# SelvinSelbaraju/hm-retrieval-two-tower

Measured on AMD Instinct MI355X. Metric: positive pairs/sec (train) + index QPS @ Recall@100, 1/2/4/8 MI355X, higher is better.
Workload: dtype bf16; 1 GPU; C3: main.py schema @ emb 128, towers [256]->128, logQ in-batch softmax, Adagrad, batch 16384; global_batch=16384, parallelism=dp1

## Files before the change

### hm-retrieval-two-tower_amd/csrc/tt_sparse.hip

```cpp
#include <algorithm>
#include <cstdlib>
#include <cstring>
#include <rocprim/device/device_radix_sort.hpp>

#include "tt_common.h"

namespace tt {
namespace {

template <char OP>
__device__ __forceinline__ float ieee_op(float a, float b) {
  if constexpr (OP == '+') return a + b;
  if constexpr (OP == '-') return a - b;
  if constexpr (OP == '*') return a * b;
  return a / b;
}

constexpr int kBlock = 32;
constexpr int kTablesPerLaunch = 16;
constexpr int kThreads = 256;
constexpr int kPFJoin = 32;
constexpr int64_t kMaxLookups = int64_t(1) << 24;
constexpr int kSrcShift = 28;

constexpr uint32_t kHdrMagic = 0x54545350u;
constexpr int kHdrBytes = 256;
enum : uint32_t { kErrStaleKeys = 1u, kErrOutOfCall = 2u };
struct SparseHeader {
  uint32_t magic;
  uint32_t error;
  uint32_t fp0, fp1;
};

struct TableDesc {
  const int32_t* ids[TT_MAX_SOURCES];
  int32_t goff[TT_MAX_SOURCES];
  const float* grad;
  int32_t gld;
  float* table;
  float* slot0;
  float* slot1;
  int64_t num_rows;
  int32_t dim;
  int32_t num_sources;
  int32_t n;
  int32_t base;
  int32_t n_pad;
  int32_t lanes;
  int32_t wave_begin;
  int32_t chunk_begin;
  int64_t piece_off;
};

struct Job {
  TableDesc t[kTablesPerLaunch];
  int32_t num;
  int32_t id_bits;
  int64_t batch;
  uint32_t* keys_in;
  uint32_t* vals_in;
  const uint32_t* keys;
  const uint32_t* vals;
  float* pieces;
  uint32_t* chunk_hist;
  int32_t num_chunks;
  float* dense_out;
  int32_t dense_dim;
  SparseHeader* hdr;
  uint32_t fp0, fp1;
};

__device__ __forceinline__ bool keys_are_mine(const Job& j) {
  const uint32_t f0 = __builtin_amdgcn_readfirstlane(__hip_atomic_load(&j.hdr->fp0, __ATOMIC_RELAXED,
                                                                        __HIP_MEMORY_SCOPE_AGENT));
  const uint32_t f1 = __builtin_amdgcn_readfirstlane(__hip_atomic_load(&j.hdr->fp1, __ATOMIC_RELAXED,
                                                                        __HIP_MEMORY_SCOPE_AGENT));
  if (f0 == j.fp0 && f1 == j.fp1) return true;
  if (lane_id() == 0) atomicOr(&j.hdr->error, kErrStaleKeys);
  return false;
}

enum ApplyOp { kWriteSum = 0, kAdagrad = 1, kAdamScatter = 2, kScatterSum = 3 };

struct ApplyParams {
  float lr;
  float eps;
  float one_minus_beta1;
  float one_minus_beta2;
};

__device__ __forceinline__ int table_of_wave(const Job& j, int gw) {
  int t = 0;
#pragma unroll 1
  for (int i = 1; i < j.num; ++i)
    if (gw >= j.t[i].wave_begin) t = i;
  return t;
}

__global__ void __launch_bounds__(kThreads) build_keys_kernel(const Job j, int total) {
  const int i = blockIdx.x * kThreads + threadIdx.x;
  if (i >= total) return;
  int t = 0;
#pragma unroll 1
  for (int k = 1; k < j.num; ++k)
    if (i >= j.t[k].base) t = k;
  const TableDesc& T = j.t[t];
  const int loc = i - T.base;
  const uint32_t invalid = (1u << j.id_bits) - 1u;
  uint32_t id = invalid, val = 0xFFFFFFFFu;
  if (loc < T.n) {
    const int s = static_cast<int>(loc / j.batch);
    const int64_t b = loc - s * j.batch;
    const int32_t r = T.ids[s][b];
    const bool ok = r >= 0 && r < T.num_rows;
    id = ok ? static_cast<uint32_t>(r) : invalid;
    val = ok ? (static_cast<uint32_t>(s) << kSrcShift) | static_cast<uint32_t>(b) : 0xFFFFFFFFu;
  }
  j.keys_in[i] = (static_cast<uint32_t>(t) << j.id_bits) | id;
  j.vals_in[i] = val;
  if (i == 0) {
    if (j.hdr->magic != kHdrMagic) {
      j.hdr->error = 0u;
      j.hdr->magic = kHdrMagic;
    }
    j.hdr->fp0 = j.fp0;
    j.hdr->fp1 = j.fp1;
  }
}

constexpr int kLdsSortMax = 16384;
constexpr int kLsThreads = 1024;
constexpr int kLsWaves = kLsThreads / kWave;
constexpr int kLsTiles = kLdsSortMax / kLsWaves / kWave;
constexpr int kHistStride = kLsWaves + 1;
constexpr int kLsLdsBytes = kLdsSortMax * 4 + 2 * kLdsSortMax * 2 + 256 * kHistStride * 4;

struct Region {
  const int32_t *ids0, *ids1, *ids2, *ids3;
  int64_t batch;
  uint32_t* keys;
  uint32_t* vals;
  int n;
  uint32_t nr;
  uint32_t khi;
  uint32_t invalid;
};

__device__ __forceinline__ int source_of(const Region& R, int64_t i) {
  return (i >= R.batch) + (i >= 2 * R.batch) + (i >= 3 * R.batch);
}

__device__ __forceinline__ uint32_t region_key(const Region& R, int i) {
// ... 91 lines not shown
  for (int u = 0; u < 4; ++u) {
    hist[hist_word(4 * tid + u)] = ex;
    ex += h[u];
  }
  __syncthreads();
}

__global__ void __launch_bounds__(kLsThreads) region_sort_kernel(const Job j) {
  extern __shared__ __attribute__((aligned(16))) char lsm[];
  uint32_t* lkey = reinterpret_cast<uint32_t*>(lsm);
  uint16_t* const pbuf0 = reinterpret_cast<uint16_t*>(lsm + kLdsSortMax * 4);
  uint16_t* const pbuf1 = pbuf0 + kLdsSortMax;
  uint32_t* hist = reinterpret_cast<uint32_t*>(lsm + kLdsSortMax * 8);
  __shared__ uint32_t wsum[kLsWaves];
  const int tid = threadIdx.x, lane = lane_id(), w = tid / kWave;
  Region R;
  int n;
  {
    const TableDesc& T = j.t[blockIdx.x];
    R.ids0 = T.ids[0];
    R.ids1 = T.ids[1];
    R.ids2 = T.ids[2];
    R.ids3 = T.ids[3];
    R.batch = j.batch;
    R.keys = const_cast<uint32_t*>(j.keys) + T.base;
    R.vals = const_cast<uint32_t*>(j.vals) + T.base;
    R.n = T.n;
    R.nr = static_cast<uint32_t>(T.num_rows);
    R.khi = static_cast<uint32_t>(blockIdx.x) << j.id_bits;
    R.invalid = (1u << j.id_bits) - 1u;
    n = T.n_pad;
  }
  const uint32_t nr = R.nr;
  if (blockIdx.x == 0 && tid == 0) {
    if (j.hdr->magic != kHdrMagic) {
      j.hdr->error = 0u;
      j.hdr->magic = kHdrMagic;
    }
    j.hdr->fp0 = j.fp0;
    j.hdr->fp1 = j.fp1;
  }
  const int bits = 32 - __builtin_clz(nr);
  const int per = ((n + kLsWaves - 1) / kLsWaves + kWave - 1) / kWave * kWave;
  const int wbeg = w * per, wend = min(n, wbeg + per);
  const uint64_t lt = (uint64_t(1) << lane) - 1u;
  for (int e = tid; e < 256 * kHistStride; e += kLsThreads) hist[e] = 0u;
  if (bits <= 8) {
    uint8_t* k8 = reinterpret_cast<uint8_t*>(lsm);
    const bool staged = n <= kLdsSortMax * 8;
    if (staged) stage_keys(R, n, k8);
    __syncthreads();
    for (int t0 = wbeg; t0 < wend; t0 += kWave) {
      const int i = t0 + lane;
      const bool act = i < wend;
      const uint32_t d = act ? (staged ? k8[i] : region_key(R, i)) : 0u;
      count_peers(hist, d, digit_peers(d, act, bits), w);
    }
    scan_digit_counts(hist, wsum);
    for (int t0 = wbeg; t0 < wend; t0 += kWave) {
      const int i = t0 + lane;
      const bool act = i < wend;
      const uint32_t d = act ? (staged ? k8[i] : region_key(R, i)) : 0u;
      const uint64_t m = digit_peers(d, act, bits);
      if (act) {
        uint32_t* slot = &hist[d * kHistStride + w];
        const uint32_t off = *slot;
// ... 101 lines not shown
    run += h[u];
  }
  uint32_t inc = run;
#pragma unroll
  for (int o = 1; o < kWave; o <<= 1) {
    const uint32_t y = __shfl_up(inc, o, kWave);
    if (lane >= o) inc += y;
  }
  if (lane == kWave - 1) wsum[w] = inc;
  __syncthreads();
  uint32_t ex = inc - run;
  for (int v = 0; v < w; ++v) ex += wsum[v];
#pragma unroll
  for (int u = 0; u < 4; ++u) {
    const int L = 4 * tid + u;
    hist[(L / kCsWaves) * kCsHistStride + L % kCsWaves] = ex;
    ex += h[u];
  }
  __syncthreads();
}

__global__ void __launch_bounds__(kCsThreads) chunk_sort_kernel(const Job j) {
  __shared__ uint32_t lkey[kChunk];
  __shared__ uint16_t pbuf[2][kChunk];
  __shared__ uint32_t hist[256 * kCsHistStride];
  __shared__ uint32_t wsum[kCsWaves];
  const int tid = threadIdx.x, lane = lane_id(), w = tid / kWave;
  const int t = table_of_chunk(j, blockIdx.x);
  const Region R = region_of(j, t);
  const int c0 = (static_cast<int>(blockIdx.x) - j.t[t].chunk_begin) * kChunk;
  const int n = min(kChunk, j.t[t].n_pad - c0);
  uint32_t* ck = j.keys_in + j.t[t].base + c0;
  uint32_t* cp = j.vals_in + j.t[t].base + c0;
  if (blockIdx.x == 0 && tid == 0) {
    if (j.hdr->magic != kHdrMagic) {
      j.hdr->error = 0u;
      j.hdr->magic = kHdrMagic;
    }
    j.hdr->fp0 = j.fp0;
    j.hdr->fp1 = j.fp1;
  }
  {
    uint32_t k[kCsTiles];
#pragma unroll
    for (int u = 0; u < kCsTiles; ++u) k[u] = region_key(R, c0 + u * kCsThreads + tid);
#pragma unroll
    for (int u = 0; u < kCsTiles; ++u) {
      const int i = u * kCsThreads + tid;
      if (i < n) {
        lkey[i] = k[u];
        pbuf[0][i] = static_cast<uint16_t>(i);
      }
    }
  }
  for (int e = tid; e < 256 * kCsHistStride; e += kCsThreads) hist[e] = 0u;
  const int bits = 32 - __builtin_clz(R.nr);
  const int per = ((n + kCsWaves - 1) / kCsWaves + kWave - 1) / kWave * kWave;
  const int wbeg = w * per, wend = min(n, wbeg + per);
  const uint64_t lt = (uint64_t(1) << lane) - 1u;
  const int passes = (bits + 7) / 8;
  const int width = (bits + passes - 1) / passes;
  const uint32_t dmask = (1u << width) - 1u;
  int cur = 0;
  for (int p = 0; p < passes; ++p) {
    const int sh = p * width;
    if (p > 0)
// ... 142 lines not shown
}

struct RowState {
  float x0, x1;
};

template <int OP>
__device__ __forceinline__ RowState load_row(const TableDesc& T, int64_t o) {
  RowState r{0.0f, 0.0f};
  if (OP == kAdagrad) {
    r.x0 = T.slot0[o];
    r.x1 = T.table[o];
  } else if (OP == kAdamScatter) {
    r.x0 = T.slot0[o];
    r.x1 = T.slot1[o];
  }
  return r;
}

template <int OP>
__device__ __forceinline__ void store_row(const TableDesc& T, const ApplyParams& ap, int64_t o, RowState r, float g) {
  if (OP == kAdagrad) {
    const float a = ieee_op<'+'>(r.x0, ieee_op<'*'>(g, g));
    T.slot0[o] = a;
    T.table[o] = ieee_op<'-'>(r.x1, ieee_op<'/'>(ieee_op<'*'>(ap.lr, g), ieee_op<'+'>(sqrtf(a), ap.eps)));
  } else if (OP == kAdamScatter) {
    T.slot0[o] = ieee_op<'+'>(r.x0, ieee_op<'*'>(g, ap.one_minus_beta1));
    T.slot1[o] = ieee_op<'+'>(r.x1, ieee_op<'*'>(ieee_op<'*'>(g, g), ap.one_minus_beta2));
  } else if (OP == kScatterSum) {
    T.table[o] = g;
  }
}

template <int OP>
__device__ __forceinline__ void apply_row(const Job& j, const TableDesc& T, const ApplyParams& ap, uint32_t key,
                                          int seg_start_sorted, int col, float g) {
  const uint32_t id = key & ((1u << j.id_bits) - 1u);
  if (OP == kWriteSum) {
    j.dense_out[static_cast<int64_t>(seg_start_sorted) * j.dense_dim + col] = g;
    return;
  }
  if (id >= static_cast<uint32_t>(T.num_rows)) return;
  const int64_t o = static_cast<int64_t>(id) * T.dim + col;
  store_row<OP>(T, ap, o, load_row<OP>(T, o), g);
}

template <int OP>
__global__ void __launch_bounds__(kThreads) block_sum_kernel(const Job j, const ApplyParams ap) {
  const int gw = __builtin_amdgcn_readfirstlane(static_cast<int>(blockIdx.x * (kThreads / kWave) + threadIdx.x / kWave));
  const int t = table_of_wave(j, gw);
  const TableDesc& T = j.t[t];
  const int P = T.lanes;
  const int lane = lane_id();
  const int blk = (gw - T.wave_begin) * (kWave / P) + lane / P;
  const int nblk = T.n_pad / kBlock;
  if (blk >= nblk) return;
  const int b0 = T.base + blk * kBlock;
  const int tend = T.base + T.n_pad;
  const uint32_t id_mask = (1u << j.id_bits) - 1u;
  uint32_t key[kBlock], off[kBlock];
#pragma unroll
  for (int r = 0; r < kBlock; ++r) {
    key[r] = j.keys[b0 + r];
    off[r] = j.vals[b0 + r];
  }
  const uint32_t kprev = blk > 0 ? j.keys[b0 - 1] : ~0u;
  const uint32_t knext = b0 + kBlock < tend ? j.keys[b0 + kBlock] : ~0u;
  if (!keys_are_mine(j)) return;
  const uint32_t gld = static_cast<uint32_t>(T.gld);
  const uint32_t go0 = T.goff[0], go1 = T.goff[1], go2 = T.goff[2], go3 = T.goff[3];
  const float* __restrict__ grad = T.grad;
  uint32_t ends = 0, apply = 0;
  bool out_of_call = false;
#pragma unroll
  for (int r = 0; r < kBlock; ++r) {
    const uint32_t s = off[r] >> kSrcShift;
    const uint32_t b = off[r] & ((1u << kSrcShift) - 1u);
    const uint32_t o = b * gld + (s == 0 ? go0 : s == 1 ? go1 : s == 2 ? go2 : go3);
    const bool in = s < static_cast<uint32_t>(T.num_sources) && b < static_cast<uint32_t>(j.batch);
    out_of_call = out_of_call || (off[r] != 0xFFFFFFFFu && !in);
    off[r] = (off[r] != 0xFFFFFFFFu && in) ? o : 0xFFFFFFFFu;
    if (r == kBlock - 1 || key[r + 1] != key[r]) ends |= 1u << r;
  }
  if (out_of_call) {
    atomicOr(&j.hdr->error, kErrOutOfCall);
    return;
  }
  const bool head_cont = key[0] == kprev;
  const bool tail_cont = key[kBlock - 1] == knext;
  {
    int seg_begin = 0;
#pragma unroll
    for (int r = 0; r < kBlock; ++r) {
      if (ends >> r & 1u) {
        const bool piece = (seg_begin == 0 && head_cont) || (r == kBlock - 1 && tail_cont);
        const bool valid = OP == kWriteSum || (key[r] & id_mask) < static_cast<uint32_t>(T.num_rows);
        if (!piece && valid) apply |= 1u << r;
        seg_begin = r + 1;
      }
    }
  }
  float* pc = j.pieces + T.piece_off + static_cast<int64_t>(blk) * 2 * T.dim;
  for (int col = lane % P; col < T.dim; col += P) {
    float v[kBlock];
#pragma unroll
    for (int r = 0; r < kBlock; ++r) v[r] = off[r] != 0xFFFFFFFFu ? grad[off[r] + col] : 0.0f;
    float acc = 0.0f;
    int seg_begin = 0;
#pragma unroll
    for (int r = 0; r < kBlock; ++r) {
      acc = ieee_op<'+'>(acc, v[r]);
      v[r] = acc;
      if (ends >> r & 1u) {
        if (seg_begin == 0 && head_cont) pc[col] = acc;
        else if (r == kBlock - 1 && tail_cont) pc[T.dim + col] = acc;
        acc = 0.0f;
        seg_begin = r + 1;
      }
    }
    if (OP == kWriteSum) {
      int sb = 0;
#pragma unroll
      for (int r = 0; r < kBlock; ++r) {
        if (apply >> r & 1u) j.dense_out[static_cast<int64_t>(b0 + sb) * j.dense_dim + col] = ieee_op<'+'>(0.0f, v[r]);
        if (ends >> r & 1u) sb = r + 1;
      }
    } else {
      RowState st[kBlock];
#pragma unroll
      for (int r = 0; r < kBlock; ++r)
        if (apply >> r & 1u) st[r] = load_row<OP>(T, static_cast<int64_t>(key[r] & id_mask) * T.dim + col);
      __builtin_amdgcn_s_waitcnt(0x0F70);
#pragma unroll
      for (int r = 0; r < kBlock; ++r)
        if (apply >> r & 1u)
          store_row<OP>(T, ap, static_cast<int64_t>(key[r] & id_mask) * T.dim + col, st[r], ieee_op<'+'>(0.0f, v[r]));
    }
  }
}

template <int OP>
__global__ void __launch_bounds__(kThreads) join_kernel(const Job j, const ApplyParams ap) {
  const int gw = __builtin_amdgcn_readfirstlane(static_cast<int>(blockIdx.x * (kThreads / kWave) + threadIdx.x / kWave));
  const int t = table_of_wave(j, gw);
  const TableDesc& T = j.t[t];
  const int P = T.lanes;
  const int lane = lane_id();
  const int blk = (gw - T.wave_begin) * (kWave / P) + lane / P;
  const int nblk = T.n_pad / kBlock;
  if (blk >= nblk) return;
  const int b0 = T.base + blk * kBlock;
  const int tend = T.base + T.n_pad;
  const uint32_t klast = j.keys[b0 + kBlock - 1];
  const uint32_t knext = b0 + kBlock < tend ? j.keys[b0 + kBlock] : ~0u;
  const bool mine = keys_are_mine(j);
  if (!mine || knext != klast) return;
  uint32_t key[kBlock];
#pragma unroll
  for (int r = 0; r < kBlock; ++r) key[r] = j.keys[b0 + r];
  const uint32_t kprev = blk > 0 ? j.keys[b0 - 1] : ~0u;
  if ((klast & ((1u << j.id_bits) - 1u)) >= static_cast<uint32_t>(T.num_rows)) return;
  int seg_start = kBlock - 1;
#pragma unroll
  for (int r = kBlock - 2; r >= 0; --r)
    if (key[r] == klast && seg_start == r + 1) seg_start = r;
  if (seg_start == 0 && kprev == klast) return;
  int lo = b0 + kBlock, hi = tend;
  {
    const int li = lane % P, g0 = lane - li;
    const uint64_t gmask = (P == kWave) ? ~0ull : (((1ull << P) - 1ull) << g0);
    while (hi - lo > 1) {
      const int step = (hi - lo + P) / (P + 1);
      const int p = lo + (li + 1) * step;
      const bool eq = p < hi && j.keys[p] == klast;
      const int c = __popcll(__ballot(eq) & gmask);
      const int nlo = lo + c * step;
      if (c < P && lo + (c + 1) * step < hi) hi = lo + (c + 1) * step;
      lo = nlo;
    }
  }
  const int last = (lo - T.base) / kBlock;
  const float* pcs = j.pieces + T.piece_off;
  for (int col = lane % P; col < T.dim; col += P) {
    float g = ieee_op<'+'>(0.0f, pcs[static_cast<int64_t>(blk) * 2 * T.dim + T.dim + col]);
    for (int bb = blk + 1; bb <= last; bb += kPFJoin) {
      float v[kPFJoin];
#pragma unroll
      for (int q = 0; q < kPFJoin; ++q)
        v[q] = (bb + q <= last) ? pcs[static_cast<int64_t>(bb + q) * 2 * T.dim + col] : 0.0f;
#pragma unroll
      for (int q = 0; q < kPFJoin; ++q)
        if (bb + q <= last) g = ieee_op<'+'>(g, v[q]);
    }
    apply_row<OP>(j, T, ap, klast, b0 + seg_start, col, g);
  }
}

__global__ void __launch_bounds__(1024) compact_kernel(const Job j, int32_t* out_uniq, float* out_sum,
                                                       int32_t* out_count) {
  const TableDesc& T = j.t[0];
  __shared__ int scratch[17];
  const int n = T.n_pad;
  const uint32_t mask = (1u << j.id_bits) - 1u;
  const int per = (n + 1023) / 1024;
  const int r0 = threadIdx.x * per, r1 = min(r0 + per, n);
  int heads = 0;
  for (int i = r0; i < r1; ++i) {
    const uint32_t k = j.keys[i];
    if ((k & mask) < static_cast<uint32_t>(T.num_rows) && (i == 0 || j.keys[i - 1] != k)) ++heads;
  }
  const int lane = lane_id(), w = threadIdx.x / kWave;
  int x = heads;
#pragma unroll
  for (int off = 1; off < kWave; off <<= 1) {
    const int y = __shfl_up(x, off, kWave);
    if (lane >= off) x += y;
  }
  if (lane == kWave - 1) scratch[w] = x;
  __syncthreads();
  if (threadIdx.x == 0) {
    int run = 0;
    for (int i = 0; i < 16; ++i) {
      const int tt = scratch[i];
      scratch[i] = run;
      run += tt;
    }
    scratch[16] = run;
// ... 42 lines not shown
  for (int i = 0; i < cnt; ++i) max_rows = std::max<int64_t>(max_rows, tables[i].num_rows);
  j.id_bits = bits_for(max_rows);
  const int table_bits = bits_for(std::max(cnt - 1, 1));
  p->end_bit = j.id_bits + table_bits;
  if (p->end_bit > 32) return fail(TT_ERR_UNSUPPORTED, "sparse: %d tables x %lld rows exceed 32-bit keys", cnt,
                                   static_cast<long long>(max_rows));
  int base = 0, waves = 0, chunks = 0;
  int64_t poff = 0;
  for (int i = 0; i < cnt; ++i) {
    const tt_sparse_table& s = tables[i];
    TableDesc& T = j.t[i];
    for (int q = 0; q < TT_MAX_SOURCES; ++q) {
      T.ids[q] = (q < s.num_sources) ? s.ids[q] : nullptr;
      T.goff[q] = (q < s.num_sources) ? s.grad_col_offset[q] : 0;
    }
    T.grad = s.grad ? s.grad : grad;
    T.gld = static_cast<int32_t>(s.grad ? s.grad_ld : grad_stride);
    if (batch > 0 && !T.grad && !size_query) return fail(TT_ERR_BAD_ARG, "sparse: table %d has no gradient (NULL grad)", i);
    int32_t max_off = 0;
    for (int q = 0; q < s.num_sources; ++q) max_off = std::max(max_off, s.grad_col_offset[q]);
    const int64_t gld = s.grad ? s.grad_ld : grad_stride;
    if (gld < 0 || max_off < 0 || (batch > 0 && (batch - 1) * gld + max_off + s.dim >= (int64_t(1) << 31)))
      return fail(TT_ERR_UNSUPPORTED, "sparse: table %d gradient rows exceed 2^31 floats", i);
    T.table = s.table;
    T.slot0 = s.slot0;
    T.slot1 = s.slot1;
    T.num_rows = s.num_rows;
    T.dim = s.dim;
    T.num_sources = s.num_sources;
    T.n = static_cast<int32_t>(s.num_sources * batch);
    T.base = base;
    T.n_pad = static_cast<int32_t>(round_up(std::max<int64_t>(T.n, 1), kBlock));
    T.lanes = lanes_per_slot(s.dim);
    T.wave_begin = waves;
    T.chunk_begin = chunks;
    T.piece_off = poff;
    base += T.n_pad;
    chunks += static_cast<int>(ceil_div(T.n_pad, kChunk));
    const int nblk = T.n_pad / kBlock;
    waves += static_cast<int>(ceil_div(nblk, kWave / T.lanes));
    poff += static_cast<int64_t>(nblk) * 2 * s.dim;
  }
  p->total = base;
  p->waves = waves;
  j.num_chunks = chunks;
  p->piece_floats = poff;
  uint32_t h0 = 2166136261u, h1 = 0x9747b28cu;
  auto mix = [&](uint64_t v) {
    for (int b = 0; b < 8; ++b) {
      const uint32_t byte = static_cast<uint32_t>(v >> (8 * b)) & 0xFFu;
      h0 = (h0 ^ byte) * 16777619u;
      h1 = (h1 ^ (byte + 0x5bu)) * 0x01000193u + 0x3c6ef372u;
    }
  };
  mix(static_cast<uint64_t>(batch));
  mix(static_cast<uint64_t>(cnt));
  for (int i = 0; i < cnt; ++i) {
    const tt_sparse_table& s = tables[i];
    mix(reinterpret_cast<uintptr_t>(s.table));
    mix(static_cast<uint64_t>(s.num_rows));
    mix((static_cast<uint64_t>(s.dim) << 32) | static_cast<uint32_t>(s.num_sources));
    for (int q = 0; q < s.num_sources; ++q) mix(reinterpret_cast<uintptr_t>(s.ids[q]));
  }
  j.fp0 = h0;
  j.fp1 = h1;
  size_t sb = 0;
  uint32_t* np = nullptr;
  hipError_t e = rocprim::radix_sort_pairs<SortConfig>(nullptr, sb, np, np, np, np, static_cast<unsigned>(base), 0, p->end_bit,
                                           nullptr, false);
  p->sort_bytes = (e == hipSuccess) ? sb : static_cast<size_t>(base) * 8 + (size_t(4) << 20);
  return TT_OK;
}

struct PlanWs {
  SparseHeader* hdr;
  uint32_t *keys_in, *vals_in, *keys, *vals;
  float* pieces;
  uint32_t* chunk_hist;
  float* dense_out;
  void* sort_tmp;
};
PlanWs carve_plan(Carver& cv, const Plan& p, int dense_dim) {
  PlanWs w;
  w.hdr = reinterpret_cast<SparseHeader*>(cv.take<char>(kHdrBytes));
  w.keys_in = cv.take<uint32_t>(p.total);
  w.vals_in = cv.take<uint32_t>(p.total);
  w.keys = cv.take<uint32_t>(p.total);
  w.vals = cv.take<uint32_t>(p.total);
  w.pieces = cv.take<float>(std::max<int64_t>(p.piece_floats, 1));
  w.chunk_hist = cv.take<uint32_t>(static_cast<int64_t>(p.job.num_chunks) * 256);
  w.dense_out = dense_dim > 0 ? cv.take<float>(static_cast<int64_t>(p.total) * dense_dim) : nullptr;
  w.sort_tmp = cv.take<char>(static_cast<int64_t>(p.sort_bytes) + 256);
  return w;
}

int validate_tables(const tt_sparse_table* tables, int32_t num_tables, int64_t batch, bool adam,
                    bool need_slot0 = true) {
  TT_REQUIRE(tables != nullptr && num_tables >= 1, "sparse: no tables");
  TT_REQUIRE(batch >= 0, "sparse: negative batch");
  int64_t total = 0;
  for (int i = 0; i < num_tables; ++i) {
    const tt_sparse_table& t = tables[i];
    TT_REQUIRE(t.table && (t.slot0 || !need_slot0), "sparse: table %d has NULL parameter/slot pointer", i);
    TT_REQUIRE(!adam || t.slot1, "sparse: table %d needs slot1 for Adam", i);
    TT_REQUIRE(t.num_rows >= 1 && t.num_rows < (int64_t(1) << 30), "sparse: table %d num_rows out of range", i);
    TT_REQUIRE(t.dim >= 1 && t.dim <= 4096, "sparse: table %d dim=%d out of range", i, t.dim);
    TT_REQUIRE(t.num_sources >= 1 && t.num_sources <= TT_MAX_SOURCES, "sparse: table %d num_sources=%d", i,
               t.num_sources);
    for (int s = 0; s < t.num_sources; ++s) TT_REQUIRE(t.ids[s] || batch == 0, "sparse: table %d source %d ids NULL", i, s);
    total += t.num_sources * batch;
  }
  TT_REQUIRE(total < kMaxLookups, "sparse: %lld lookups in one call (max %lld)", static_cast<long long>(total),
             static_cast<long long>(kMaxLookups));
  return TT_OK;
}

size_t tables_ws_bytes(const tt_sparse_table* tables, int32_t num_tables, int64_t batch, int dense_dim) {
  size_t total = 0;
  for (int first = 0; first < num_tables; first += kTablesPerLaunch) {
    const int cnt = std::min(num_tables - first, kTablesPerLaunch);
    Plan p;
    if (make_plan(tables + first, cnt, batch, nullptr, 0, &p, true)) return 0;
// ... 10 lines not shown
    const char* e = std::getenv("TT_SPARSE_SORT");
    if (e && std::strcmp(e, "device") == 0) return int(kSortDevice);
    if (e && std::strcmp(e, "region") == 0) return int(kSortRegion);
    return int(kSortChunk);
  }();
  return v;
}

enum SparseStage { kStageAll = 0, kStageSort = 1, kStageApply = 2 };

template <int OP>
int run_sparse(const tt_sparse_table* tables, int32_t num_tables, int64_t batch, const float* grad,
               int64_t grad_stride, const ApplyParams& ap, void* workspace, size_t ws_bytes, hipStream_t st,
               int32_t* out_uniq = nullptr, float* out_sum = nullptr, int32_t* out_count = nullptr,
               int stage = kStageAll) {
  TT_REQUIRE(batch < (int64_t(1) << kSrcShift), "sparse: batch %lld too large", static_cast<long long>(batch));
  TT_REQUIRE(stage == kStageAll || num_tables <= kTablesPerLaunch,
             "sparse: a split sort/apply call takes at most %d tables", kTablesPerLaunch);
  for (int first = 0; first < num_tables; first += kTablesPerLaunch) {
    const int cnt = std::min(num_tables - first, kTablesPerLaunch);
    Plan p;
    int rc = make_plan(tables + first, cnt, batch, grad, grad_stride, &p, stage == kStageSort);
    if (rc) return rc;
    Carver cv(workspace, ws_bytes);
    const int dense_dim = (OP == kWriteSum) ? tables[first].dim : 0;
    PlanWs w = carve_plan(cv, p, dense_dim);
    if (cv.used() > ws_bytes) return fail(TT_ERR_WORKSPACE, "sparse: workspace %zu < required %zu", ws_bytes, cv.used());
    Job& j = p.job;
    j.keys_in = w.keys_in;
    j.vals_in = w.vals_in;
    j.keys = w.keys;
    j.vals = w.vals;
    j.pieces = w.pieces;
    j.chunk_hist = w.chunk_hist;
    j.dense_out = w.dense_out;
    j.dense_dim = dense_dim;
    j.hdr = w.hdr;
    if (stage != kStageApply) {
      const int mode = sort_mode();
      bool lds = mode != kSortDevice, chunked = mode == kSortChunk;
      int merge_chunks = 0;
      for (int i = 0; i < cnt; ++i) {
        const bool small = bits_for(j.t[i].num_rows) <= 8;
        lds = lds && (j.t[i].n_pad <= kLdsSortMax || small);
        chunked = chunked && (small ? j.t[i].n_pad <= kChunkMaxSmall : j.t[i].n_pad <= kChunkMaxLarge);
        if (!small) merge_chunks = std::max(merge_chunks, static_cast<int>(ceil_div(j.t[i].n_pad, kChunk)));
      }
      if (chunked) {
        hipLaunchKernelGGL(chunk_sort_kernel, dim3(j.num_chunks), dim3(kCsThreads), 0, st, j);
        TT_CHECK_LAUNCH();
        static const hipError_t attr = hipFuncSetAttribute(reinterpret_cast<const void*>(chunk_merge_kernel),
                                                           hipFuncAttributeMaxDynamicSharedMemorySize, kMergeLdsMax);
        TT_CHECK_HIP(attr);
        hipLaunchKernelGGL(chunk_merge_kernel, dim3(j.num_chunks), dim3(kCsThreads), merge_chunks * kChunk * 4, st,
                           j);
        TT_CHECK_LAUNCH();
      } else if (lds) {
        static const hipError_t attr = hipFuncSetAttribute(reinterpret_cast<const void*>(region_sort_kernel),
                                                           hipFuncAttributeMaxDynamicSharedMemorySize, kLsLdsBytes);
        TT_CHECK_HIP(attr);
        hipLaunchKernelGGL(region_sort_kernel, dim3(cnt), dim3(kLsThreads), kLsLdsBytes, st, j);
        TT_CHECK_LAUNCH();
      } else {
        hipLaunchKernelGGL(build_keys_kernel, dim3(ceil_div(p.total, kThreads)), dim3(kThreads), 0, st, j, p.total);
        TT_CHECK_LAUNCH();
        size_t sb = p.sort_bytes;
        TT_CHECK_HIP(rocprim::radix_sort_pairs<SortConfig>(w.sort_tmp, sb, w.keys_in, w.keys, w.vals_in, w.vals,
                                               static_cast<unsigned>(p.total), 0, p.end_bit, st, false));
      }
    }
    if (stage == kStageSort) continue;
    const int blocks = static_cast<int>(ceil_div(p.waves, kThreads / kWave));
    hipLaunchKernelGGL(block_sum_kernel<OP>, dim3(blocks), dim3(kThreads), 0, st, j, ap);
    TT_CHECK_LAUNCH();
    hipLaunchKernelGGL(join_kernel<OP>, dim3(blocks), dim3(kThreads), 0, st, j, ap);
    TT_CHECK_LAUNCH();
    if (OP == kWriteSum) {
      hipLaunchKernelGGL(compact_kernel, dim3(1), dim3(1024), 0, st, j, out_uniq, out_sum, out_count);
      TT_CHECK_LAUNCH();
    }
  }
  return TT_OK;
}

__global__ void scale2_kernel(float* a, float sa, float* b, float sb, int64_t n) {
  for (int64_t i = blockIdx.x * (int64_t)blockDim.x + threadIdx.x; i < n; i += (int64_t)gridDim.x * blockDim.x) {
    a[i] = ieee_op<'*'>(a[i], sa);
    b[i] = ieee_op<'*'>(b[i], sb);
  }
}

__global__ void adam_var_kernel(float* var, const float* m, const float* v, float lr, float eps, int64_t n) {
  for (int64_t i = blockIdx.x * (int64_t)blockDim.x + threadIdx.x; i < n; i += (int64_t)gridDim.x * blockDim.x)
    var[i] = ieee_op<'-'>(var[i], ieee_op<'/'>(ieee_op<'*'>(lr, m[i]), ieee_op<'+'>(sqrtf(v[i]), eps)));
}

__global__ void dense_adagrad_kernel(float* p, float* acc, const float* g, int64_t n, float lr, float eps) {
  for (int64_t i = blockIdx.x * (int64_t)blockDim.x + threadIdx.x; i < n; i += (int64_t)gridDim.x * blockDim.x) {
    const float gi = g[i];
    const float a = ieee_op<'+'>(acc[i], ieee_op<'*'>(gi, gi));
    acc[i] = a;
    p[i] = ieee_op<'-'>(p[i], ieee_op<'/'>(ieee_op<'*'>(gi, lr), ieee_op<'+'>(sqrtf(a), eps)));
  }
}

constexpr int kDenseMaxJobs = 8;
struct DenseJobs {
  float* p[kDenseMaxJobs];
  float* acc[kDenseMaxJobs];
// ... 123 lines not shown
    for (int q = 0; q < w; ++q) ex += wsum[q];
    if (tid < r.world) pre[tid * T + t] = ex;
  }
  __syncthreads();
  const int64_t i = static_cast<int64_t>(blockIdx.x) * kRoutedThreads + tid;
  const uint32_t invalid = (1u << j.id_bits) - 1u;
  if (i < r.total) {
    const int lk = r.order[i];
    const int l = static_cast<int>(lk / j.batch);
    const int b = static_cast<int>(lk - static_cast<int64_t>(l) * j.batch);
    const int s = r.slot[lk];
    const int o = s >= 0 ? static_cast<int>(s / r.cap) : -1 - s;
    const int g = o * T + r.lk_tag[l];
    const int dst = r.lk_base[l] + pre[g] + static_cast<int>(i - r.grp_first[g]);
    uint32_t id = s >= 0 ? static_cast<uint32_t>(s) : invalid;
    if (r.slot_row && s >= 0) {
      const int32_t row = r.slot_row[s];
      id = row >= 0 ? static_cast<uint32_t>(row) : invalid;
    }
    const_cast<uint32_t*>(j.keys)[dst] = r.lk_khi[l] | id;
    const_cast<uint32_t*>(j.vals)[dst] = id == invalid ? 0xFFFFFFFFu : (r.lk_shi[l] | static_cast<uint32_t>(b));
  } else {
    const int k = static_cast<int>(i - r.total);
    int t = 0;
#pragma unroll 1
    for (int q = 1; q < r.num_tables; ++q)
      if (k >= r.pad_begin[q]) t = q;
    if (k < r.pad_begin[r.num_tables]) {
      const int dst = r.pad_dst[t] + (k - r.pad_begin[t]);
      const_cast<uint32_t*>(j.keys)[dst] = r.pad_key[t];
      const_cast<uint32_t*>(j.vals)[dst] = 0xFFFFFFFFu;
    }
  }
  if (i == 0) {
    if (j.hdr->magic != kHdrMagic) {
      j.hdr->error = 0u;
      j.hdr->magic = kHdrMagic;
    }
    j.hdr->fp0 = j.fp0;
    j.hdr->fp1 = j.fp1;
  }
}

dim3 stride_grid(int64_t n) {
  int64_t b = ceil_div(n, 256);
  if (b > 8192) b = 8192;
  if (b < 1) b = 1;
  return dim3(static_cast<unsigned>(b));
}

}
}

using namespace tt;

extern "C" size_t tt_sparse_workspace_size(const tt_sparse_table* tables, int32_t num_tables, int64_t batch) {
  if (!tables || num_tables < 1 || batch < 0) return 0;
  return tables_ws_bytes(tables, num_tables, batch, 0);
}

namespace tt {
namespace {
int sparse_adagrad_stage(const tt_sparse_table* tables, int32_t num_tables, int64_t batch, const float* grad,
                         int64_t grad_stride, float lr, float epsilon, void* workspace, size_t workspace_bytes,
                         tt_stream_t stream, int stage, const char* name) {
  clear_error();
// ... 241 lines not shown
  TT_REQUIRE(L >= 1 && L <= kRoutedMaxLookups, "tt_sparse_routed: 1..%d lookups, got %d", kRoutedMaxLookups, L);
  TT_REQUIRE(W >= 1 && W <= kRoutedThreads && T >= 1 && static_cast<int64_t>(W) * T <= kRoutedMaxGroups,
             "tt_sparse_routed: world %d x tags %d out of range", W, T);
  TT_REQUIRE(rs->cap >= 1, "tt_sparse_routed: cap must be >= 1");
  int tag_of_table[kTablesPerLaunch], seen[kTablesPerLaunch][TT_MAX_SOURCES] = {};
  for (int t = 0; t < num_tables; ++t) tag_of_table[t] = -1;
  for (int l = 0; l < L; ++l) {
    const int t = rs->lookup_table[l], s = rs->lookup_source[l], g = rs->lookup_tag[l];
    TT_REQUIRE(t >= 0 && t < num_tables && s >= 0 && s < tables[t].num_sources && g >= 0 && g < T,
               "tt_sparse_routed: lookup %d maps to table %d source %d tag %d: out of range", l, t, s, g);
    TT_REQUIRE(tag_of_table[t] < 0 || tag_of_table[t] == g, "tt_sparse_routed: table %d takes two tags", t);
    TT_REQUIRE(!seen[t][s], "tt_sparse_routed: table %d source %d listed twice", t, s);
    tag_of_table[t] = g;
    seen[t][s] = 1;
  }
  for (int t = 0; t < num_tables; ++t)
    for (int s = 0; s < tables[t].num_sources; ++s)
      TT_REQUIRE(seen[t][s], "tt_sparse_routed: table %d source %d has no routed lookup", t, s);
  for (int t = 0; t < num_tables; ++t)
    for (int u = t + 1; u < num_tables; ++u)
      TT_REQUIRE(tag_of_table[t] != tag_of_table[u], "tt_sparse_routed: tables %d and %d take one tag", t, u);
  const size_t need = tables_ws_bytes(tables, num_tables, batch, 0);
  if (!workspace || workspace_bytes < need)
    return fail(TT_ERR_WORKSPACE, "tt_sparse_routed: workspace %zu < required %zu", workspace_bytes, need);
  TT_REQUIRE(batch < (int64_t(1) << kSrcShift), "tt_sparse_routed: batch too large");
  Plan p;
  rc = make_plan(tables, num_tables, batch, grad, grad_stride, &p);
  if (rc) return rc;
  Carver cv(workspace, workspace_bytes);
  PlanWs w = carve_plan(cv, p, 0);
  Job& j = p.job;
  j.keys = w.keys;
  j.vals = w.vals;
  j.hdr = w.hdr;
  RoutedArgs a{};
  a.order = rs->order;
  a.grp_first = rs->grp_first;
  a.grp_last = rs->grp_last;
  a.slot = rs->slot;
  a.slot_row = rs->slot_row;
  a.cap = rs->cap;
  a.total = static_cast<int64_t>(L) * batch;
  a.world = W;
  a.num_tags = T;
  a.num_lookups = L;
  a.num_tables = num_tables;
  for (int l = 0; l < L; ++l) {
    const int t = rs->lookup_table[l];
    a.lk_tag[l] = rs->lookup_tag[l];
    a.lk_khi[l] = static_cast<uint32_t>(t) << j.id_bits;
    a.lk_shi[l] = static_cast<uint32_t>(rs->lookup_source[l]) << kSrcShift;
    a.lk_base[l] = j.t[t].base;
  }
  int pads = 0;
  for (int t = 0; t < num_tables; ++t) {
    a.pad_begin[t] = pads;
    a.pad_dst[t] = j.t[t].base + j.t[t].n;
    a.pad_key[t] = (static_cast<uint32_t>(t) << j.id_bits) | ((1u << j.id_bits) - 1u);
    pads += j.t[t].n_pad - j.t[t].n;
  }
  a.pad_begin[num_tables] = pads;
  TT_REQUIRE(a.total + pads == p.total, "tt_sparse_routed: %lld routed lookups + %d padding != %d sorted entries",
             static_cast<long long>(a.total), pads, p.total);
  hipStream_t st = to_stream(stream);
  hipLaunchKernelGGL(routed_keys_kernel, dim3(static_cast<unsigned>(ceil_div(p.total, kRoutedThreads))),
                     dim3(kRoutedThreads), 0, st, j, a);
// ... 28 lines not shown
```

Measured before the change: 32.03 million positive pairs/s.

## Fuse cross-block segment join into block_sum via arrival counters

Removes the separate join_kernel launch. Segments that span several 32-row blocks are now finished by whichever block arrives last, tracked with per-block atomic arrival counters that are reset in the key-building and sort kernels. The segment-extent search runs forward and backward at once. Wave assignment now puts small tables (<=255 rows) first, presumably so their long, contended segments start early. This saves a kernel launch and a full pass over keys, but adds atomics, relaxed-memory publish/read of partial sums, and a new workspace array, with some risk around memory ordering.

```diff
diff --git a/hm-retrieval-two-tower_amd/csrc/tt_sparse.hip b/hm-retrieval-two-tower_amd/csrc/tt_sparse.hip
--- a/hm-retrieval-two-tower_amd/csrc/tt_sparse.hip
+++ b/hm-retrieval-two-tower_amd/csrc/tt_sparse.hip
@@ -20,6 +20,8 @@
 constexpr int kTablesPerLaunch = 16;
 constexpr int kThreads = 256;
 constexpr int kPFJoin = 32;
+constexpr int kPFShort = 4;
+constexpr int kSmallRows = 255;
 constexpr int64_t kMaxLookups = int64_t(1) << 24;
 constexpr int kSrcShift = 28;
 
@@ -62,6 +64,7 @@
   const uint32_t* keys;
   const uint32_t* vals;
   float* pieces;
+  uint32_t* arrived;
   uint32_t* chunk_hist;
   int32_t num_chunks;
   float* dense_out;
@@ -90,10 +93,15 @@
 };
 
 __device__ __forceinline__ int table_of_wave(const Job& j, int gw) {
-  int t = 0;
+  int t = 0, best = -1;
 #pragma unroll 1
-  for (int i = 1; i < j.num; ++i)
-    if (gw >= j.t[i].wave_begin) t = i;
+  for (int i = 0; i < j.num; ++i) {
+    const int wb = j.t[i].wave_begin;
+    if (gw >= wb && wb > best) {
+      t = i;
+      best = wb;
+    }
+  }
   return t;
 }
 
@@ -118,6 +126,7 @@
   }
   j.keys_in[i] = (static_cast<uint32_t>(t) << j.id_bits) | id;
   j.vals_in[i] = val;
+  if (i % kBlock == 0) j.arrived[i / kBlock] = 0u;
   if (i == 0) {
     if (j.hdr->magic != kHdrMagic) {
       j.hdr->error = 0u;
@@ -275,6 +284,7 @@
     n = T.n_pad;
   }
   const uint32_t nr = R.nr;
+  for (int e = tid; e < n / kBlock; e += kLsThreads) j.arrived[j.t[blockIdx.x].base / kBlock + e] = 0u;
   if (blockIdx.x == 0 && tid == 0) {
     if (j.hdr->magic != kHdrMagic) {
       j.hdr->error = 0u;
@@ -442,6 +452,7 @@
   const int n = min(kChunk, j.t[t].n_pad - c0);
   uint32_t* ck = j.keys_in + j.t[t].base + c0;
   uint32_t* cp = j.vals_in + j.t[t].base + c0;
+  if (tid < n / kBlock) j.arrived[(j.t[t].base + c0) / kBlock + tid] = 0u;
   if (blockIdx.x == 0 && tid == 0) {
     if (j.hdr->magic != kHdrMagic) {
       j.hdr->error = 0u;
@@ -650,17 +661,60 @@
   }
 }
 
+__device__ __forceinline__ void publish_piece(float* p, float v) {
+  __hip_atomic_store(p, v, __ATOMIC_RELAXED, __HIP_MEMORY_SCOPE_AGENT);
+}
+__device__ __forceinline__ float read_piece(const float* p) {
+  return __hip_atomic_load(p, __ATOMIC_RELAXED, __HIP_MEMORY_SCOPE_AGENT);
+}
+
+template <int N>
+__device__ __forceinline__ void add_pieces(const float* pcs, int dim, int i0, int n, int col, int col1, float& g0,
+                                           float& g1) {
+  float v0[N], v1[N];
+#pragma unroll
+  for (int q = 0; q < N; ++q) {
+    const int i = min(i0 + q, n);
+    const float* p = pcs + static_cast<int64_t>(i) * 2 * dim + (i == 0 ? dim : 0);
+    v0[q] = read_piece(p + col);
+    v1[q] = read_piece(p + col1);
+  }
+#pragma unroll
+  for (int q = 0; q < N; ++q) {
+    const bool in = i0 + q <= n;
+    g0 = in ? ieee_op<'+'>(g0, v0[q]) : g0;
+    g1 = in ? ieee_op<'+'>(g1, v1[q]) : g1;
+  }
+}
+
 template <int OP>
-__device__ __forceinline__ void apply_row(const Job& j, const TableDesc& T, const ApplyParams& ap, uint32_t key,
-                                          int seg_start_sorted, int col, float g) {
-  const uint32_t id = key & ((1u << j.id_bits) - 1u);
-  if (OP == kWriteSum) {
-    j.dense_out[static_cast<int64_t>(seg_start_sorted) * j.dense_dim + col] = g;
-    return;
-  }
-  if (id >= static_cast<uint32_t>(T.num_rows)) return;
-  const int64_t o = static_cast<int64_t>(id) * T.dim + col;
-  store_row<OP>(T, ap, o, load_row<OP>(T, o), g);
+__device__ __forceinline__ void join_segment(const Job& j, const TableDesc& T, const ApplyParams& ap, uint32_t key,
+                                             int seg_start_sorted, int first, int last, int P, int li) {
+  const float* pcs = j.pieces + T.piece_off + static_cast<int64_t>(first) * 2 * T.dim;
+  const int dim = T.dim, n = last - first;
+  const int64_t row = static_cast<int64_t>(key & ((1u << j.id_bits) - 1u)) * dim;
+  for (int col = li; col < dim; col += 2 * P) {
+    const bool two = col + P < dim;
+    const int col1 = two ? col + P : col;
+    RowState r0{0.0f, 0.0f}, r1{0.0f, 0.0f};
+    if (OP != kWriteSum) {
+      r0 = load_row<OP>(T, row + col);
+      r1 = load_row<OP>(T, row + col1);
+    }
+    float g0 = 0.0f, g1 = 0.0f;
+    if (n < kPFShort) {
+      add_pieces<kPFShort>(pcs, dim, 0, n, col, col1, g0, g1);
+    } else {
+      for (int i0 = 0; i0 <= n; i0 += kPFJoin) add_pieces<kPFJoin>(pcs, dim, i0, n, col, col1, g0, g1);
+    }
+    if (OP == kWriteSum) {
+      j.dense_out[static_cast<int64_t>(seg_start_sorted) * j.dense_dim + col] = g0;
+      if (two) j.dense_out[static_cast<int64_t>(seg_start_sorted) * j.dense_dim + col1] = g1;
+    } else {
+      store_row<OP>(T, ap, row + col, r0, g0);
+      if (two) store_row<OP>(T, ap, row + col1, r1, g1);
+    }
+  }
 }
 
 template <int OP>
@@ -674,7 +728,6 @@
   const int nblk = T.n_pad / kBlock;
   if (blk >= nblk) return;
   const int b0 = T.base + blk * kBlock;
-  const int tend = T.base + T.n_pad;
   const uint32_t id_mask = (1u << j.id_bits) - 1u;
   uint32_t key[kBlock], off[kBlock];
 #pragma unroll
@@ -682,9 +735,15 @@
     key[r] = j.keys[b0 + r];
     off[r] = j.vals[b0 + r];
   }
-  const uint32_t kprev = blk > 0 ? j.keys[b0 - 1] : ~0u;
-  const uint32_t knext = b0 + kBlock < tend ? j.keys[b0 + kBlock] : ~0u;
-  if (!keys_are_mine(j)) return;
+  const int li = lane % P;
+  const uint64_t gmask = (P == kWave) ? ~0ull : (((1ull << P) - 1ull) << (lane - li));
+  const int nfwd = nblk - 1 - blk, nbwd = blk;
+  const uint32_t fk0 = j.keys[b0 + (li < nfwd ? kBlock * (1 + li) : 0)];
+  const uint32_t bk0 = j.keys[b0 - (li < nbwd ? 1 + kBlock * li : 0)];
+  const bool mine = keys_are_mine(j);
+  int flo = __popcll(__ballot(li < nfwd && fk0 == key[kBlock - 1]) & gmask);
+  int blo = __popcll(__ballot(li < nbwd && bk0 == key[0]) & gmask);
+  if (!mine) return;
   const uint32_t gld = static_cast<uint32_t>(T.gld);
   const uint32_t go0 = T.goff[0], go1 = T.goff[1], go2 = T.goff[2], go3 = T.goff[3];
   const float* __restrict__ grad = T.grad;
@@ -704,8 +763,8 @@
     atomicOr(&j.hdr->error, kErrOutOfCall);
     return;
   }
-  const bool head_cont = key[0] == kprev;
-  const bool tail_cont = key[kBlock - 1] == knext;
+  const bool head_cont = blo > 0;
+  const bool tail_cont = flo > 0;
   {
     int seg_begin = 0;
 #pragma unroll
@@ -730,8 +789,8 @@
       acc = ieee_op<'+'>(acc, v[r]);
       v[r] = acc;
       if (ends >> r & 1u) {
-        if (seg_begin == 0 && head_cont) pc[col] = acc;
-        else if (r == kBlock - 1 && tail_cont) pc[T.dim + col] = acc;
+        if (seg_begin == 0 && head_cont) publish_piece(&pc[col], acc);
+        else if (r == kBlock - 1 && tail_cont) publish_piece(&pc[T.dim + col], acc);
         acc = 0.0f;
         seg_begin = r + 1;
       }
@@ -755,62 +814,51 @@
           store_row<OP>(T, ap, static_cast<int64_t>(key[r] & id_mask) * T.dim + col, st[r], ieee_op<'+'>(0.0f, v[r]));
     }
   }
-}
-
-template <int OP>
-__global__ void __launch_bounds__(kThreads) join_kernel(const Job j, const ApplyParams ap) {
-  const int gw = __builtin_amdgcn_readfirstlane(static_cast<int>(blockIdx.x * (kThreads / kWave) + threadIdx.x / kWave));
-  const int t = table_of_wave(j, gw);
-  const TableDesc& T = j.t[t];
-  const int P = T.lanes;
-  const int lane = lane_id();
-  const int blk = (gw - T.wave_begin) * (kWave / P) + lane / P;
-  const int nblk = T.n_pad / kBlock;
-  if (blk >= nblk) return;
-  const int b0 = T.base + blk * kBlock;
-  const int tend = T.base + T.n_pad;
-  const uint32_t klast = j.keys[b0 + kBlock - 1];
-  const uint32_t knext = b0 + kBlock < tend ? j.keys[b0 + kBlock] : ~0u;
-  const bool mine = keys_are_mine(j);
-  if (!mine || knext != klast) return;
-  uint32_t key[kBlock];
-#pragma unroll
-  for (int r = 0; r < kBlock; ++r) key[r] = j.keys[b0 + r];
-  const uint32_t kprev = blk > 0 ? j.keys[b0 - 1] : ~0u;
-  if ((klast & ((1u << j.id_bits) - 1u)) >= static_cast<uint32_t>(T.num_rows)) return;
-  int seg_start = kBlock - 1;
-#pragma unroll
-  for (int r = kBlock - 2; r >= 0; --r)
-    if (key[r] == klast && seg_start == r + 1) seg_start = r;
-  if (seg_start == 0 && kprev == klast) return;
-  int lo = b0 + kBlock, hi = tend;
-  {
-    const int li = lane % P, g0 = lane - li;
-    const uint64_t gmask = (P == kWave) ? ~0ull : (((1ull << P) - 1ull) << g0);
-    while (hi - lo > 1) {
-      const int step = (hi - lo + P) / (P + 1);
-      const int p = lo + (li + 1) * step;
-      const bool eq = p < hi && j.keys[p] == klast;
-      const int c = __popcll(__ballot(eq) & gmask);
-      const int nlo = lo + c * step;
-      if (c < P && lo + (c + 1) * step < hi) hi = lo + (c + 1) * step;
-      lo = nlo;
-    }
-  }
-  const int last = (lo - T.base) / kBlock;
-  const float* pcs = j.pieces + T.piece_off;
-  for (int col = lane % P; col < T.dim; col += P) {
-    float g = ieee_op<'+'>(0.0f, pcs[static_cast<int64_t>(blk) * 2 * T.dim + T.dim + col]);
-    for (int bb = blk + 1; bb <= last; bb += kPFJoin) {
-      float v[kPFJoin];
-#pragma unroll
-      for (int q = 0; q < kPFJoin; ++q)
-        v[q] = (bb + q <= last) ? pcs[static_cast<int64_t>(bb + q) * 2 * T.dim + col] : 0.0f;
-#pragma unroll
-      for (int q = 0; q < kPFJoin; ++q)
-        if (bb + q <= last) g = ieee_op<'+'>(g, v[q]);
-    }
-    apply_row<OP>(j, T, ap, klast, b0 + seg_start, col, g);
+  const uint32_t rows = static_cast<uint32_t>(T.num_rows);
+  const uint32_t kf = key[kBlock - 1], kb = key[0];
+  const bool whole = ends == 1u << (kBlock - 1);
+  const bool head_seg = head_cont && (kb & id_mask) < rows;
+  const bool fwd = tail_cont && (kf & id_mask) < rows;
+  const bool tail_seg = fwd && !(whole && head_cont);
+  if (!head_seg && !fwd) return;
+  int fhi = (fwd && flo == P) ? nfwd : flo, bhi = (head_seg && blo == P) ? nbwd : blo;
+  while (fhi > flo || bhi > blo) {
+    const int fs = (fhi - flo + P) / (P + 1) + (fhi == flo), bs = (bhi - blo + P) / (P + 1) + (bhi == blo);
+    const int fp = flo - 1 + (li + 1) * fs, bp = blo - 1 + (li + 1) * bs;
+    const bool fin = fp < fhi, bin = bp < bhi;
+    const uint32_t fk = j.keys[b0 + (fin ? kBlock * (1 + fp) : 0)], bk = j.keys[b0 - (bin ? 1 + kBlock * bp : 0)];
+    const int fc = __popcll(__ballot(fin && fk == kf) & gmask);
+    const int bc = __popcll(__ballot(bin && bk == kb) & gmask);
+    if (fc < P && flo + (fc + 1) * fs - 1 < fhi) fhi = flo + (fc + 1) * fs - 1;
+    if (bc < P && blo + (bc + 1) * bs - 1 < bhi) bhi = blo + (bc + 1) * bs - 1;
+    flo += fc * fs;
+    blo += bc * bs;
+  }
+  const int last = blk + flo;
+  const int first = blk - blo;
+  const int head_last = (whole && fwd) ? last : blk;
+  const int tail_start = kBlock - __clz(ends & ~(1u << (kBlock - 1)));
+  asm volatile("s_waitcnt vmcnt(0)" ::: "memory");
+  uint32_t* arrived = j.arrived + T.base / kBlock;
+  uint32_t th = ~0u, tk = ~0u;
+  if (li == 0 && head_seg) th = __hip_atomic_fetch_add(&arrived[first], 1u, __ATOMIC_RELAXED, __HIP_MEMORY_SCOPE_AGENT);
+  if (li == 0 && tail_seg) tk = __hip_atomic_fetch_add(&arrived[blk], 1u, __ATOMIC_RELAXED, __HIP_MEMORY_SCOPE_AGENT);
+  const bool join_head = (__ballot(th == static_cast<uint32_t>(head_last - first)) & gmask) != 0;
+  const bool join_tail = (__ballot(tk == static_cast<uint32_t>(last - blk)) & gmask) != 0;
+  __builtin_amdgcn_fence(__ATOMIC_ACQUIRE, "wavefront");
+#pragma unroll 1
+  for (int s = 0; s < 2; ++s) {
+    if (!(s == 0 ? join_head : join_tail)) continue;
+    const int f = s == 0 ? first : blk;
+    int start_sorted = b0 + tail_start;
+    if (OP == kWriteSum && s == 0) {
+      int same = 0;
+      for (int r = li; r - li < kBlock; r += P)
+        same += __popcll(__ballot(r < kBlock && j.keys[T.base + f * kBlock + min(r, kBlock - 1)] == kb) & gmask);
+      start_sorted = T.base + (f + 1) * kBlock - same;
+    }
+    join_segment<OP>(j, T, ap, s == 0 ? kb : kf, start_sorted, f, s == 0 ? head_last : last, P, li);
+    if (li == 0) __hip_atomic_store(&arrived[f], 0u, __ATOMIC_RELAXED, __HIP_MEMORY_SCOPE_AGENT);
   }
 }
 
@@ -919,15 +967,19 @@
     T.base = base;
     T.n_pad = static_cast<int32_t>(round_up(std::max<int64_t>(T.n, 1), kBlock));
     T.lanes = lanes_per_slot(s.dim);
-    T.wave_begin = waves;
     T.chunk_begin = chunks;
     T.piece_off = poff;
     base += T.n_pad;
     chunks += static_cast<int>(ceil_div(T.n_pad, kChunk));
-    const int nblk = T.n_pad / kBlock;
-    waves += static_cast<int>(ceil_div(nblk, kWave / T.lanes));
-    poff += static_cast<int64_t>(nblk) * 2 * s.dim;
-  }
+    poff += static_cast<int64_t>(T.n_pad / kBlock) * 2 * s.dim;
+  }
+  for (int pass = 0; pass < 2; ++pass)
+    for (int i = 0; i < cnt; ++i) {
+      TableDesc& T = j.t[i];
+      if ((T.num_rows <= kSmallRows) != (pass == 0)) continue;
+      T.wave_begin = waves;
+      waves += static_cast<int>(ceil_div(T.n_pad / kBlock, kWave / T.lanes));
+    }
   p->total = base;
   p->waves = waves;
   j.num_chunks = chunks;
@@ -963,6 +1015,7 @@
   SparseHeader* hdr;
   uint32_t *keys_in, *vals_in, *keys, *vals;
   float* pieces;
+  uint32_t* arrived;
   uint32_t* chunk_hist;
   float* dense_out;
   void* sort_tmp;
@@ -975,6 +1028,7 @@
   w.keys = cv.take<uint32_t>(p.total);
   w.vals = cv.take<uint32_t>(p.total);
   w.pieces = cv.take<float>(std::max<int64_t>(p.piece_floats, 1));
+  w.arrived = cv.take<uint32_t>(p.total / kBlock);
   w.chunk_hist = cv.take<uint32_t>(static_cast<int64_t>(p.job.num_chunks) * 256);
   w.dense_out = dense_dim > 0 ? cv.take<float>(static_cast<int64_t>(p.total) * dense_dim) : nullptr;
   w.sort_tmp = cv.take<char>(static_cast<int64_t>(p.sort_bytes) + 256);
@@ -1051,6 +1105,7 @@
     j.keys = w.keys;
     j.vals = w.vals;
     j.pieces = w.pieces;
+    j.arrived = w.arrived;
     j.chunk_hist = w.chunk_hist;
     j.dense_out = w.dense_out;
     j.dense_dim = dense_dim;
@@ -1092,8 +1147,6 @@
     const int blocks = static_cast<int>(ceil_div(p.waves, kThreads / kWave));
     hipLaunchKernelGGL(block_sum_kernel<OP>, dim3(blocks), dim3(kThreads), 0, st, j, ap);
     TT_CHECK_LAUNCH();
-    hipLaunchKernelGGL(join_kernel<OP>, dim3(blocks), dim3(kThreads), 0, st, j, ap);
-    TT_CHECK_LAUNCH();
     if (OP == kWriteSum) {
       hipLaunchKernelGGL(compact_kernel, dim3(1), dim3(1024), 0, st, j, out_uniq, out_sum, out_count);
       TT_CHECK_LAUNCH();
@@ -1283,6 +1336,7 @@
       const_cast<uint32_t*>(j.vals)[dst] = 0xFFFFFFFFu;
     }
   }
+  if (i < r.total + r.pad_begin[r.num_tables] && i % kBlock == 0) j.arrived[i / kBlock] = 0u;
   if (i == 0) {
     if (j.hdr->magic != kHdrMagic) {
       j.hdr->error = 0u;
@@ -1590,6 +1644,7 @@
   Job& j = p.job;
   j.keys = w.keys;
   j.vals = w.vals;
+  j.arrived = w.arrived;
   j.hdr = w.hdr;
   RoutedArgs a{};
   a.order = rs->order;
```

New measurement: 32.46 million positive pairs/s, median of 6. +1.4%, better.
